# vkit-x/vkit

Measured on AMD Instinct MI355X. Metric: Mpixels/s (2048^2 RGB, geo+photo chain), higher is better.
Workload: dtype u8; 1 GPU; C3 fused chain: camera_cubic_curve remap (level 5) + gaussian_blur(sigma=1.0) + color_shift(37) + gaussion_noise(std=10.0, the numpy stream default_rng(5000 + i) drawn on the device inside every step), states built from the configs inside every step, 2048x2048x3 uint8, batch 256 per GPU; batch_per_gpu=256, image=2048x2048x3, noise_mode=tiles, states=built on the device from the configs inside every step (vkx_camera_states_dev), lanes=1

## Files before the change

vkit_amd/csrc/chain.hip:

```cpp
#include "vkx_internal.h"

#include <stdlib.h>
#include <algorithm>
#include <memory>
#include <unordered_map>
#include <vector>

static int chain_check_items(const vkx_chain_item *items, int n_items)
{
    for (int i = 0; i < n_items; i++) {
        const vkx_chain_item &it = items[i];
        VKX_REQUIRE(it.src && it.dst && it.src_vertices && it.dst_vertices, "NULL plane in chain item");
        VKX_REQUIRE(it.sh > 0 && it.sw > 0 && it.dh > 0 && it.dw > 0, "bad shape in chain item");
        VKX_REQUIRE_PITCH(it.src_stride, (ptrdiff_t)it.sw * 3, it.sh);
        VKX_REQUIRE_PITCH(it.dst_stride, (ptrdiff_t)it.dw * 3, it.dh);
        if (it.noise && !it.noise_tiled) VKX_REQUIRE_PITCH(it.noise_stride_el, (ptrdiff_t)it.dw * 3, it.dh);
        VKX_REQUIRE_DISJOINT(it.src, it.sh, it.src_stride, (size_t)it.sw * 3, it.dst, it.dh, it.dst_stride, (size_t)it.dw * 3);
        if (it.streak_enabled) {
            VKX_REQUIRE(it.streak_thickness + it.streak_gap > 0, "streak thickness + gap must be positive");
            if (it.streak_alpha < 0.0 || it.streak_alpha > 1.0) {
                vkx_set_error("alpha=%g is invalid.", it.streak_alpha);
                return VKX_ERR_INVALID;
            }
        }
// ... 112 lines not shown
        rc = vkx_chain_plan_build(ctx, items, n_items, &raw);
        if (rc && rc != VKX_ERR_UNSUPPORTED) return rc;
    }
    if (!raw) {
        if ((rc = vkx_chain_consume_lattices_mark(ctx))) return rc;
        if ((rc = vkx_np_draw_batch_dev(ctx, jobs, n_jobs, results_host))) return rc;
        return vkx_chain_rgb_batch_dev(ctx, items, n_items);
    }
    std::unique_ptr<vkx_chain_plan, void (*)(vkx_chain_plan *)> plan(raw, vkx_chain_plan_free);
    const int n_chunks = std::max(1, std::min(want_chunks, n_jobs / 8));
    struct Chunk { int job0, njobs, item0, nitems; vkx_np_chunk *np; hipEvent_t posted; };
    std::vector<Chunk> chunks((size_t)n_chunks);
    for (int c = 0; c < n_chunks; c++) {
        Chunk &ch = chunks[c];
        ch.job0 = (int)((long long)n_jobs * c / n_chunks);
        ch.njobs = (int)((long long)n_jobs * (c + 1) / n_chunks) - ch.job0;
        ch.item0 = c == 0 ? 0 : job_item[ch.job0];
        ch.np = nullptr; ch.posted = nullptr;
    }
    for (int c = 0; c < n_chunks; c++) chunks[c].nitems = (c + 1 < n_chunks ? chunks[c + 1].item0 : n_items) - chunks[c].item0;
    struct Cleanup {
        std::vector<Chunk> &chunks;
        ~Cleanup() { for (Chunk &ch : chunks) { if (ch.np) vkx_np_chunk_free(ch.np); if (ch.posted) (void)hipEventDestroy(ch.posted); } }
    } cleanup{chunks};

    vkx_device_guard guard(ctx);
    hipStream_t main_stream = ctx->stream;
    const char *fail_env = getenv("VKX_DEBUG_FAIL_CHUNK");
    const int fail_chunk = fail_env && fail_env[0] ? atoi(fail_env) : -1;
    auto schedule = [&]() -> int {
        int rc = VKX_OK;
        hipStream_t aux = vkx_stream_by_id(ctx, VKX_STREAM_COPY_IN, &rc);
        if (rc) return rc;
        hipEvent_t setup_done = nullptr;
        if ((rc = vkx_chain_plan_setup_aside(ctx, raw, &setup_done))) return rc;
        if (setup_done) VKX_HIP(hipStreamWaitEvent(aux, setup_done, 0));
        for (int c = 0; c < n_chunks; c++) {
            Chunk &ch = chunks[c];
            if (c >= 2) VKX_HIP(hipStreamWaitEvent(main_stream, chunks[c - 2].posted, 0));
            if ((rc = vkx_np_chunk_begin(ctx, jobs + ch.job0, ch.njobs, results_host + ch.job0, c & 1, &ch.np))) return rc;
            if ((rc = vkx_stream_order(ctx, aux, main_stream))) return rc;
            ctx->stream = aux;
            rc = vkx_np_chunk_finish(ctx, ch.np);
            if (!rc) rc = vkx_chain_plan_noise_rows(ctx, raw, ch.item0, ch.nitems);
            ctx->stream = main_stream;
            if (rc) return rc;
            VKX_HIP(hipEventCreateWithFlags(&ch.posted, hipEventDisableTiming));
            VKX_HIP(hipEventRecord(ch.posted, aux));
            if (c == fail_chunk) {
                vkx_set_error("injected failure in chunk %d (VKX_DEBUG_FAIL_CHUNK)", c);
                return VKX_ERR_INVALID;
            }
        }
        if (setup_done) VKX_HIP(hipStreamWaitEvent(main_stream, setup_done, 0));
        for (int c = 0; c < n_chunks; c++) {
            Chunk &ch = chunks[c];
            VKX_HIP(hipStreamWaitEvent(main_stream, ch.posted, 0));
            if ((rc = vkx_chain_plan_tiles(ctx, raw, ch.item0, ch.nitems))) return rc;
        }
        return vkx_chain_mark_done(ctx, main_stream);
    };
    rc = schedule();
    if (rc) vkx_ctx_join_streams(ctx, main_stream);
    return rc;
}
```

vkit_amd/csrc/ctx.hip:

```cpp
#include "vkx_internal.h"

#include <stdarg.h>
#include <stdio.h>

static thread_local char g_err[512] = "";

void vkx_set_error(const char *fmt, ...)
{
    va_list ap;
    va_start(ap, fmt);
    vsnprintf(g_err, sizeof g_err, fmt, ap);
    va_end(ap);
}

VKX_EXPORT const char *vkx_last_error(void) { return g_err; }
VKX_EXPORT int vkx_version(void) { return 1; }

VKX_EXPORT int vkx_device_count(int *count)
{
    VKX_REQUIRE(count != nullptr, "count is NULL");
    VKX_HIP(hipGetDeviceCount(count));
    return VKX_OK;
}

// ... 34 lines not shown

static void scratch_release(vkx_scratch *s)
{
    if (s->ptr) (void)hipFree(s->ptr);
    s->ptr = nullptr;
    s->cap = 0;
}

VKX_EXPORT int vkx_ctx_destroy(vkx_ctx *ctx)
{
    if (!ctx) return VKX_OK;
    (void)hipSetDevice(ctx->device);
    (void)hipStreamSynchronize(ctx->stream);
    for (auto &st : ctx->copy_stream)
        if (st) (void)hipStreamSynchronize(st);
    scratch_release(&ctx->owner);
    scratch_release(&ctx->paint_owner);
    scratch_release(&ctx->cells);
    scratch_release(&ctx->misc);
    scratch_release(&ctx->tables);
    for (auto &s : ctx->stage) scratch_release(&s);
    for (auto &s : ctx->chain) scratch_release(&s);
    scratch_release(&ctx->chain_cells);
    scratch_release(&ctx->chain_bins);
    scratch_release(&ctx->chain_misc);
    if (ctx->chain_done) (void)hipEventDestroy(ctx->chain_done);
    if (ctx->chain_setup_done) (void)hipEventDestroy(ctx->chain_setup_done);
    if (ctx->lattices_ready) (void)hipEventDestroy(ctx->lattices_ready);
    scratch_release(&ctx->noise_table);
    scratch_release(&ctx->np_tabs);
    scratch_release(&ctx->noise_rows);
    scratch_release(&ctx->np_work[0]);
    scratch_release(&ctx->np_work[1]);
    scratch_release(&ctx->camera_work);
    scratch_release(&ctx->mls_work);
    scratch_release(&ctx->fog_work);
    scratch_release(&ctx->crop_windows);
    scratch_release(&ctx->crop_planes);
    scratch_release(&ctx->combine_tables);
    scratch_release(&ctx->char_table);
    scratch_release(&ctx->char_geo);
    scratch_release(&ctx->char_layout);
    scratch_release(&ctx->char_host);
    scratch_release(&ctx->char_owner);
    scratch_release(&ctx->heat_table);
    scratch_release(&ctx->heat_geo);
    scratch_release(&ctx->heat_host);
    scratch_release(&ctx->heat_planes);
    scratch_release(&ctx->rl_deviate);
    scratch_release(&ctx->rl_planes);
    scratch_release(&ctx->rc_tables);
    scratch_release(&ctx->rc_bitmap);
    scratch_release(&ctx->rf_tables);
    scratch_release(&ctx->rm_tables);
    scratch_release(&ctx->rm_bits);
    scratch_release(&ctx->set_tables);
    scratch_release(&ctx->set_planes);
    scratch_release(&ctx->seal_tables);
    scratch_release(&ctx->seal_planes);
    scratch_release(&ctx->text_tables);
    scratch_release(&ctx->text_planes);
    scratch_release(&ctx->layer_tables);
    scratch_release(&ctx->quad_tables);
    scratch_release(&ctx->collate_tables);
    scratch_release(&ctx->contour_tables);
    scratch_release(&ctx->contour_planes);
// ... 560 lines not shown
```

vkit_amd/csrc/fused.hip:

```cpp
#include "vkx_internal.h"
#include "vkx_cell.h"
#include "vkx_color.h"

#include <float.h>
#include <memory>
#include <stdlib.h>
#include <string.h>

namespace {

constexpr int W = 64;
constexpr int RMAX = 3;
constexpr int NLDSCELL = 64;
#ifndef VKX_FUSED_NWAVES
#define VKX_FUSED_NWAVES 8
#endif
constexpr int NWAVES = VKX_FUSED_NWAVES;
constexpr int NTHREADS = 64 * NWAVES;
constexpr int ROWS_PER_WAVE = 8;
constexpr int WH = NWAVES * ROWS_PER_WAVE;
__host__ __device__ constexpr int tile_side(int R) { return (W - 2 * R) & ~3; }
__host__ __device__ constexpr int tile_height(int R) { return WH == W ? tile_side(R) : WH - 2 * R; }
#ifndef VKX_FUSED_CGROUP
#define VKX_FUSED_CGROUP 2
// ... 1114 lines not shown
    rec.y = before | (step << 16);
    ((u32x2 VKX_GLOBAL *)it.noise_rows)[k] = rec;
}

__global__ void __launch_bounds__(256) k_chain_prologue(uint32_t *__restrict__ desc_dst, const uint32_t *__restrict__ desc_src,
                                                        unsigned n_words, TileBin *__restrict__ bins, unsigned nbins,
                                                        int *__restrict__ deferred, int *__restrict__ over_count, unsigned n_over)
{
    const unsigned i = blockIdx.x * 256 + threadIdx.x;
    if (i < n_words) desc_dst[i] = desc_src[i];
    if (i < nbins) bins[i] = TileBin{0x7f7f7f7f, 0x7f7f7f7f, 0, 0};
    if (i < n_over) over_count[i] = 0;
    if (i == 0) *deferred = 0;
}

}

struct vkx_chain_plan {
    std::vector<ItemDev> dev;
    std::vector<int> prefix;
    std::vector<long long> row_prefix;
    long long ncells = 0;
    int max_tiles = 0, slots = 0;
    int rect_slots = 0;
    bool elements = false, streak = false;
    const ItemDev *d_items = nullptr;
    const int *d_cell_prefix = nullptr;
    TileBin *bins = nullptr;
    vkc::CellC *cells = nullptr;
    int *deferred = nullptr;
    int *over_count = nullptr;
    int2 *over_list = nullptr;
    const HsvLut *lut = nullptr;
};

void vkx_chain_plan_free(vkx_chain_plan *p) { delete p; }
int vkx_chain_plan_items(const vkx_chain_plan *p) { return (int)p->dev.size(); }

int vkx_chain_plan_setup(vkx_ctx *ctx, vkx_chain_plan *p)
{
    const int n_items = (int)p->dev.size();
    int rc;
    vkx_scratch *s_cells = p->elements ? &ctx->cells : &ctx->chain_cells;
    vkx_scratch *s_bins = p->elements ? &ctx->owner : &ctx->chain_bins;
    vkx_scratch *s_misc = p->elements ? &ctx->misc : &ctx->chain_misc;
    const size_t cells_bytes = sizeof(vkc::CellC) * (size_t)p->ncells;
    if ((rc = vkx_scratch_reserve(ctx, s_cells, cells_bytes + sizeof(int) * ((size_t)p->ncells + 1)))) return rc;
    p->slots = ((p->max_tiles + 7) / 8) * 8;
    const size_t nbins = (size_t)p->slots * n_items;
    if (n_items > 65535) return VKX_ERR_UNSUPPORTED;
    const size_t over_ints = p->elements ? 0 : (size_t)n_items * (2 + 2 * (size_t)p->rect_slots);
    if ((rc = vkx_scratch_reserve(ctx, s_bins, sizeof(TileBin) * nbins + sizeof(int) * over_ints))) return rc;
    const size_t items_bytes = sizeof(ItemDev) * (size_t)n_items, prefix_bytes = sizeof(int) * p->prefix.size();
    vkx_tables tab(ctx);
    const size_t items_off = tab.add(items_bytes), prefix_off = tab.add(prefix_bytes), misc_bytes = tab.bytes;
    if ((rc = vkx_scratch_reserve(ctx, s_misc, misc_bytes))) return rc;
    if (!p->elements && (rc = vkx_hsv_tables(ctx, (const void **)&p->lut))) return rc;
    unsigned char *misc = (unsigned char *)s_misc->ptr;
    if ((rc = tab.take())) return rc;
    memcpy(tab.at<char>(items_off), p->dev.data(), items_bytes);
    memcpy(tab.at<char>(prefix_off), p->prefix.data(), prefix_bytes);
    p->d_items = (const ItemDev *)(misc + items_off);
    p->d_cell_prefix = (const int *)(misc + prefix_off);
    p->bins = (TileBin *)s_bins->ptr;
    p->over_count = (int *)(p->bins + nbins);
    p->over_list = (int2 *)(p->over_count + n_items + (n_items & 1));
    p->cells = (vkc::CellC *)s_cells->ptr;
    p->deferred = (int *)((unsigned char *)s_cells->ptr + cells_bytes);
    {
        const unsigned char *ring_dev = tab.mapped();
        if (!ring_dev) { vkx_set_error("%s: the descriptor ring is not mapped into the device's address space", __func__); return VKX_ERR_HIP; }
        const size_t n_words = (misc_bytes + 3) / 4;
        VKX_TIMED(ctx, "k_chain_prologue");
        k_chain_prologue<<<vkx_blocks(std::max(n_words, nbins), 256), 256, 0, ctx->stream>>>((uint32_t *)misc, (const uint32_t *)ring_dev,
                                                                                            (unsigned)n_words, p->bins, (unsigned)nbins, p->deferred,
                                                                                            p->over_count, p->elements ? 0u : (unsigned)n_items);
        VKX_LAUNCH_CHECK();
    }
    { VKX_TIMED(ctx, "k_chain_setup"); k_chain_setup<<<vkx_blocks((size_t)p->ncells, 256), 256, 0, ctx->stream>>>(p->d_items, p->d_cell_prefix, n_items, (int)p->ncells, p->slots, p->cells, p->bins, p->deferred); }
    VKX_LAUNCH_CHECK();
    { VKX_TIMED(ctx, "k_chain_setup_svd"); k_chain_setup_svd<<<128, 64, 0, ctx->stream>>>(p->d_items, p->d_cell_prefix, n_items, p->cells, p->deferred); }
    VKX_LAUNCH_CHECK();
    return VKX_OK;
}

int vkx_chain_plan_noise_rows(vkx_ctx *ctx, vkx_chain_plan *p, int first, int count)
{
    if (p->row_prefix.empty() || count <= 0) return VKX_OK;
    long long most = 0;
    for (int i = first; i < first + count; i++) most = std::max(most, p->row_prefix[i + 1] - p->row_prefix[i]);
    if (most <= 0) return VKX_OK;
    VKX_TIMED(ctx, "k_chain_noise_rows");
    k_chain_noise_rows<<<dim3(vkx_blocks((size_t)most, 256), count), 256, 0, ctx->stream>>>(p->d_items + first);
    VKX_LAUNCH_CHECK();
    return VKX_OK;
}

int vkx_chain_plan_tiles(vkx_ctx *ctx, vkx_chain_plan *p, int first, int count)
{
    if (count <= 0) return VKX_OK;
    static const int phase_limit = vkx_env_int("VKX_FUSED_PHASES", 0);
    const ItemDev *items = p->d_items + first;
    const TileBin *bins = p->bins + (size_t)first * p->slots;
    if (p->elements) {
        const dim3 grid(p->slots, count);
        VKX_TIMED(ctx, "k_tile_remap");
        ElemPack pack;
        memset(&pack, 0, sizeof(pack));
        pack.n = p->dev[first].n_elems;
        for (int e = 0; e < 4; e++) pack.el[e] = p->dev[first].el[e];
        k_tile_remap<<<grid, NTHREADS, kFusedLds, ctx->stream>>>(items, p->cells, bins, pack);
    } else {
        int most_rect = 0, most_rim = 0;
        long long all_rect = 0, all_tiles = 0;
        for (int i = first; i < first + count; i++) {
            const ItemDev &d = p->dev[i];
            most_rect = std::max(most_rect, d.rect_w * d.rect_h);
            all_rect += d.rect_w * d.rect_h;
            all_tiles += (long long)d.tiles_x * d.tiles_y;
            most_rim = std::max(most_rim, d.tiles_x * d.tiles_y - d.rect_w * d.rect_h);
        }
        int *over_count = p->over_count + first;
        int2 *over_list = p->over_list + (size_t)first * p->rect_slots;
        const int over_slots = (int)std::min<long long>((long long)count * p->rect_slots, INT_MAX);
        VKX_TIMED_MAJOR(ctx, "k_chain_fused");
        constexpr long long kSplitMinTiles = 65536;
        const int split_env = vkx_env_on("VKX_CHAIN_SPLIT", -1);
        if (split_env >= 0 ? split_env == 0 : all_tiles < kSplitMinTiles) {
            const dim3 grid(p->slots, count);
            if (p->streak) k_chain_fused_whole<true><<<grid, NTHREADS, kFusedLds, ctx->stream>>>(items, p->cells, bins, p->lut, phase_limit);
            else k_chain_fused_whole<false><<<grid, NTHREADS, kFusedLds, ctx->stream>>>(items, p->cells, bins, p->lut, phase_limit);
            VKX_LAUNCH_CHECK();
            return VKX_OK;
        }
        if (most_rect > 0) {
            const dim3 grid_rect((most_rect + 7) / 8 * 8, count);
            if (p->streak) k_chain_fused<true><<<grid_rect, NTHREADS, kFusedLds, ctx->stream>>>(items, p->cells, bins, p->slots, over_count, over_list, over_slots, p->lut, phase_limit);
            else k_chain_fused<false><<<grid_rect, NTHREADS, kFusedLds, ctx->stream>>>(items, p->cells, bins, p->slots, over_count, over_list, over_slots, p->lut, phase_limit);
            VKX_LAUNCH_CHECK();
        }
        if (most_rim > 0) {
            const dim3 grid_rim((most_rim + 7) / 8 * 8, count);
            if (p->streak) k_chain_fused_rim<true><<<grid_rim, NTHREADS, kFusedLds, ctx->stream>>>(items, p->cells, bins, p->slots, p->lut, phase_limit);
            else k_chain_fused_rim<false><<<grid_rim, NTHREADS, kFusedLds, ctx->stream>>>(items, p->cells, bins, p->slots, p->lut, phase_limit);
            VKX_LAUNCH_CHECK();
        }
        if (most_rect > 0) {
            const dim3 grid_over((unsigned)std::min<long long>((all_rect + 1) / 2, kOverGrid));
            if (p->streak) k_chain_fused_over<true><<<grid_over, NTHREADS, kFusedLds, ctx->stream>>>(items, p->cells, bins, p->slots, over_count, over_list, over_slots, p->lut, phase_limit);
            else k_chain_fused_over<false><<<grid_over, NTHREADS, kFusedLds, ctx->stream>>>(items, p->cells, bins, p->slots, over_count, over_list, over_slots, p->lut, phase_limit);
        }
    }
    VKX_LAUNCH_CHECK();
    return VKX_OK;
}

int vkx_chain_plan_build(vkx_ctx *ctx, const vkx_chain_item *items, int n_items, vkx_chain_plan **out)
{
    *out = nullptr;
    if (n_items <= 0) return VKX_OK;
    std::unique_ptr<vkx_chain_plan> plan(new vkx_chain_plan());
    std::vector<ItemDev> &dev = plan->dev;
    dev.resize(n_items);
    plan->prefix.resize((size_t)n_items + 1);
    int *cell_prefix = plan->prefix.data();
    std::vector<long long> &row_prefix = plan->row_prefix;
    row_prefix.assign((size_t)n_items + 1, 0);
    long long tiles = 0, ncells = 0;
    int max_tiles = 0, max_rect = 0;
    for (int i = 0; i < n_items; i++) {
        const vkx_chain_item &it = items[i];
        if (it.blur_ksize > 2 * RMAX + 1 || (it.blur_ksize > 1 && (it.blur_ksize & 1) == 0)) return VKX_ERR_UNSUPPORTED;
        if (it.sh > 32767 || it.sw > 32767 || it.dh > 32767 || it.dw > 32767) return VKX_ERR_UNSUPPORTED;
        if (it.rows < 2 || it.cols < 2) return VKX_ERR_UNSUPPORTED;
        if (it.blur_ksize > 1 && (it.dh == 1 || it.dw == 1)) return VKX_ERR_UNSUPPORTED;
        ItemDev &d = dev[i];
        memset(&d, 0, sizeof(d));
        d.src = it.src; d.dst = it.dst; d.noise = it.noise; d.sv = it.src_vertices; d.dv = it.dst_vertices;
        d.sstride = it.src_stride; d.dstride = it.dst_stride; d.nstride = it.noise_stride_el;
        d.noise_table = nullptr; d.noise_tiled = 0; d.noise_tiles = 0; d.noise_slot = 0; d.noise_tiles_per_sample = 0.f;
        d.noise_rows = nullptr;
        if (it.noise && it.noise_tiled) {
            const long long n = (long long)it.dh * it.dw * 3;
            if (n > 0x7fffffffLL) return VKX_ERR_UNSUPPORTED;
            const vkx_np_tiles_shape shape = vkx_np_tiles_shape_of(n);
            if (shape.n_tiles * shape.slot_elems > 0xffffffffLL) return VKX_ERR_UNSUPPORTED;
            d.noise = (const int16_t *)((const unsigned char *)it.noise + shape.slots_offset);
// ... 157 lines not shown
```

vkit_amd/csrc/nprand.hip:

```cpp
#include "vkx_internal.h"
#include "np_ziggurat.h"
#include "vkx_host_tables.h"

#include <stddef.h>
#include <string.h>
#include <algorithm>

namespace {

typedef unsigned __int128 u128;
#define VKX_GLOBAL __attribute__((address_space(1)))

#ifndef VKX_NP_ROUNDS
#define VKX_NP_ROUNDS 48
#endif
constexpr int kRounds = VKX_NP_ROUNDS;
static_assert(kRounds % 2 == 0 && kRounds >= 2 && kRounds <= 64, "rounds per tile");
constexpr int kTile = 64 * kRounds;
constexpr double kNorR = 3.6541528853610087963519472518;
constexpr double kNorInvR = 0.27366123732975827203338247596;

#define PCG_MULT VKX_PCG_MULT
using vkx_host_tables::JumpTabs;

// ... 1223 lines not shown
    bool uniform, inline_jobs;
    long long total_tiles;
    vkx_np_result *results_host, *res_mapped;
    unsigned char *base;
    size_t o_states, o_info, o_plan, o_rmask, o_rval, o_jobs, o_results;
    NpJobPack pack;
    const NpTabs *tabs;
};

static int np_chunk_prepare(vkx_ctx *ctx, NpChunk &c)
{
    const bool uniform = c.uniform;
    c.total_tiles = 0;
    c.max_tiles = 0;
    for (int i = 0; i < c.n_jobs; i++) {
        const long long tiles = np_tiles_for(c.jobs[i], uniform);
        c.max_tiles = std::max<int>(c.max_tiles, (int)tiles);
        c.total_tiles += tiles;
    }
    size_t off = 0;
    auto take = [&off](size_t bytes) { const size_t o = off; off += vkx_align256(bytes); return o; };
    c.o_states = take((size_t)c.total_tiles * 16);
    c.o_info = take(uniform ? 0 : (size_t)c.total_tiles * sizeof(TileInfo));
    c.o_plan = take(uniform ? 0 : (size_t)c.total_tiles * sizeof(TilePlan));
    const bool speckle = c.kind == VKX_NP_SPECKLE_U8;
    const bool slots = c.kind == VKX_NP_NORMAL_I16 || c.kind == VKX_NP_NORMAL_ADD_U8;
    c.o_rmask = take(speckle ? (size_t)c.total_tiles * kRounds * 8 : 0);
    c.o_rval = take(speckle ? (size_t)c.total_tiles * kTile * 8 : slots ? (size_t)c.total_tiles * kSlot * 2 : 0);
    c.o_jobs = take((size_t)c.n_jobs * sizeof(NpJob));
    c.o_results = take((size_t)c.n_jobs * sizeof(vkx_np_result) + sizeof(unsigned));
    int rc = vkx_scratch_reserve(ctx, &ctx->np_work[c.slot], off);
    if (rc) return rc;
    c.base = (unsigned char *)ctx->np_work[c.slot].ptr;

    c.inline_jobs = c.n_jobs <= kInlineJobs;
    NpJob *hj = c.pack.jobs;
    vkx_tables tab(ctx);
    if (!c.inline_jobs) {
        if ((rc = tab.take((size_t)c.n_jobs * sizeof(NpJob)))) return rc;
        hj = tab.at<NpJob>(0);
    }
    const JumpTabs &jump = vkx_host_tables::jump_tabs();
    const u128 g64 = ((u128)jump.g64[1] << 64) | jump.g64[0];
    const u128 g128 = ((u128)jump.g128[1] << 64) | jump.g128[0];
    long long tile_base = 0;
    for (int i = 0; i < c.n_jobs; i++) {
        const vkx_np_job &j = c.jobs[i];
        NpJob &d = hj[i];
        d.state[0] = j.state[0]; d.state[1] = j.state[1];
        d.inc[0] = j.inc[0]; d.inc[1] = j.inc[1];
        const u128 c64 = (((u128)j.inc[1] << 64) | j.inc[0]) * g64;
        d.c64[0] = (uint64_t)c64; d.c64[1] = (uint64_t)(c64 >> 64);
        const u128 c128 = (((u128)j.inc[1] << 64) | j.inc[0]) * g128;
        d.c128[0] = (uint64_t)c128; d.c128[1] = (uint64_t)(c128 >> 64);
        d.n = j.n;
        d.tile_base = tile_base;
        d.n_tiles = (int)np_tiles_for(j, uniform);
        tile_base += d.n_tiles;
        d.kind = j.kind & 0xff; d.cn = j.cn;
        d.margin = (j.kind & VKX_NP_DEBUG_WIDE_MARGIN) ? 1.0 : 0x1p-42;
        d.loc = 0.0; d.scale = j.scale;
        d.cdf[0] = j.cdf[0]; d.cdf[1] = j.cdf[1]; d.cdf[2] = j.cdf[2];
        d.src = (const uint8_t *)j.src;
        d.dst = j.dst;
        d.rec = nullptr;
        d.table = nullptr;
        if (c.kind == VKX_NP_NORMAL_TILES) {
            const vkx_np_tiles_shape shape = vkx_np_tiles_shape_of(j.n);
            d.rec = (int16_t *)((unsigned char *)j.dst + shape.slots_offset);
            d.table = (uint2 *)((unsigned char *)j.dst + shape.table_offset);
        } else if (slots) {
            d.rec = (int16_t *)(c.base + c.o_rval) + d.tile_base * kSlot;
        }
    }
    if (!c.inline_jobs && (rc = tab.small_to(c.base + c.o_jobs))) return rc;
    c.res_mapped = nullptr;
    if (hipHostGetDevicePointer((void **)&c.res_mapped, c.results_host, 0) != hipSuccess) {
        (void)hipGetLastError();
        c.res_mapped = nullptr;
    }
    return VKX_OK;
}

static int np_chunk_front(vkx_ctx *ctx, NpChunk &c)
{
    unsigned char *base = c.base;
    const NpJob *dj = (const NpJob *)(base + c.o_jobs);
    uint64_t *states = (uint64_t *)(base + c.o_states);
    TileInfo *info = (TileInfo *)(base + c.o_info);
    vkx_np_result *res = (vkx_np_result *)(base + c.o_results);
    unsigned *done = (unsigned *)(res + c.n_jobs);
    const long long total_tiles = c.total_tiles;
    const int n_jobs = c.n_jobs, kind = c.kind;
    const NpTabs *tabs = c.tabs;
    static const int tpw_env = vkx_env_int("VKX_NP_TPW", 0);
    const int tiles_per_wave = tpw_env > 0 ? tpw_env : (total_tiles >= 160000 ? 4 : total_tiles >= 40000 ? 2 : 1);
    const unsigned wg = (unsigned)((total_tiles + 4 * tiles_per_wave - 1) / (4 * tiles_per_wave));
    {
        VKX_TIMED(ctx, "k_np_tile_states");
        if (c.inline_jobs)
            k_np_tile_states<true><<<vkx_blocks((size_t)total_tiles, 256), 256, 0, ctx->stream>>>(dj, c.pack, n_jobs, total_tiles, states, (NpJob *)(base + c.o_jobs), res, done, tabs);
        else
            k_np_tile_states<false><<<vkx_blocks((size_t)total_tiles, 256), 256, 0, ctx->stream>>>(dj, c.pack, n_jobs, total_tiles, states, (NpJob *)(base + c.o_jobs), res, done, tabs);
        VKX_LAUNCH_CHECK();
    }
    if (c.uniform) {
        VKX_TIMED(ctx, "k_np_choice_impulse");
        k_np_choice_impulse<<<wg, 256, 0, ctx->stream>>>(dj, n_jobs, total_tiles, states, res, done, c.res_mapped, tabs);
        VKX_LAUNCH_CHECK();
        return VKX_OK;
    }
    if (np_compact_records(kind)) {
        VKX_TIMED_MAJOR(ctx, "k_np_draw");
        bool bytes = true;
        for (int i = 0; i < n_jobs; i++) bytes = bytes && np_parks_as_bytes(c.jobs[i].scale, 0.0);
        const long long waves = bytes ? DrawShape<EmitI16B8>::kWaves : DrawShape<EmitI16>::kWaves;
        const unsigned wgc = (unsigned)((total_tiles + waves * tiles_per_wave - 1) / (waves * tiles_per_wave));
        const long long run = (total_tiles + (long long)wgc * waves - 1) / ((long long)wgc * waves);
        if (bytes)
            k_np_draw_compact<EmitI16B8><<<wgc, 64 * (unsigned)waves, 0, ctx->stream>>>(dj, n_jobs, total_tiles, run, states, info, res, tabs);
        else
            k_np_draw_compact<EmitI16><<<wgc, 64 * (unsigned)waves, 0, ctx->stream>>>(dj, n_jobs, total_tiles, run, states, info, res, tabs);
        VKX_LAUNCH_CHECK();
        return VKX_OK;
    }
    VKX_TIMED_MAJOR(ctx, "k_np_draw");
    k_np_draw<EmitSpeckle><<<wg, 256, 0, ctx->stream>>>(dj, n_jobs, total_tiles, states, info, (double *)(base + c.o_rval),
                                                        (uint64_t *)(base + c.o_rmask), res, tabs);
    VKX_LAUNCH_CHECK();
    return VKX_OK;
}

static int np_chunk_back(vkx_ctx *ctx, NpChunk &c)
{
    if (c.uniform) {
        if (!c.res_mapped)
            VKX_HIP(hipMemcpyAsync(c.results_host, c.base + c.o_results, (size_t)c.n_jobs * sizeof(vkx_np_result), hipMemcpyDeviceToHost, ctx->stream));
        return VKX_OK;
// ... 78 lines not shown
            VKX_REQUIRE(uniform, "normal and uniform jobs in one call");
            break;
        case VKX_NP_IMPULSE_U8:
            VKX_REQUIRE(uniform, "normal and uniform jobs in one call");
            VKX_REQUIRE(j.src != nullptr && j.cn >= 1 && j.cn <= 4, "bad impulse job");
            break;
        default:
            VKX_REQUIRE(false, "unknown job kind");
        }
        if (!uniform) VKX_REQUIRE(j.scale >= 0.0 && j.scale < 400.0, "scale outside [0, 400)");
        VKX_REQUIRE(np_tiles_for(j, uniform) <= 262144, "stream too long for one job (2.6e8 samples)");
    }
    return VKX_OK;
}

struct vkx_np_chunk { NpChunk c; };

int vkx_np_chunk_begin(vkx_ctx *ctx, const vkx_np_job *jobs, int n_jobs, vkx_np_result *results_host, int slot, vkx_np_chunk **out)
{
    *out = nullptr;
    const NpTabs *tabs = nullptr;
    int rc = np_tables(ctx, &tabs);
    if (rc) return rc;
    vkx_np_chunk *h = new (std::nothrow) vkx_np_chunk();
    if (!h) { vkx_set_error("out of host memory"); return VKX_ERR_NOMEM; }
    NpChunk &c = h->c;
    c.jobs = jobs; c.n_jobs = n_jobs;
    c.kind = jobs[0].kind & 0xff;
    c.uniform = c.kind == VKX_NP_CHOICE3_U8 || c.kind == VKX_NP_IMPULSE_U8;
    c.slot = slot & 1;
    c.results_host = results_host;
    c.tabs = tabs;
    vkx_device_guard guard(ctx);
    if ((rc = np_chunk_prepare(ctx, c)) || (rc = np_chunk_front(ctx, c))) { delete h; return rc; }
    *out = h;
    return VKX_OK;
}

int vkx_np_chunk_finish(vkx_ctx *ctx, vkx_np_chunk *h)
{
    vkx_device_guard guard(ctx);
    return np_chunk_back(ctx, h->c);
}

void vkx_np_chunk_free(vkx_np_chunk *h) { delete h; }

VKX_EXPORT int vkx_np_draw_batch_dev(vkx_ctx *ctx, const vkx_np_job *jobs, int n_jobs, vkx_np_result *results_host)
{
    VKX_REQUIRE(ctx && jobs && results_host, "NULL argument");
    int rc = vkx_np_jobs_check(jobs, n_jobs, results_host);
    if (rc) return rc;
    const int kind = jobs[0].kind & 0xff;
    const bool uniform = kind == VKX_NP_CHOICE3_U8 || kind == VKX_NP_IMPULSE_U8;
    const NpTabs *tabs = nullptr;
    if ((rc = np_tables(ctx, &tabs))) return rc;
    vkx_device_guard guard(ctx);
    const int n_chunks = (!uniform && kind != VKX_NP_NORMAL_TILES && n_jobs >= 2 * kChunkJobs) ? (n_jobs + kChunkJobs - 1) / kChunkJobs : 1;
    auto chunk_of = [&](int k, NpChunk &c) {
        const int per = (n_jobs + n_chunks - 1) / n_chunks, first = k * per;
        c.jobs = jobs + first;
        c.n_jobs = std::min(per, n_jobs - first);
        c.kind = kind; c.uniform = uniform; c.slot = k & 1;
        c.results_host = results_host + first;
        c.tabs = tabs;
    };
    if (n_chunks == 1) {
        NpChunk c;
        chunk_of(0, c);
        if ((rc = np_chunk_prepare(ctx, c)) || (rc = np_chunk_front(ctx, c))) return rc;
        return np_chunk_back(ctx, c);
    }
    hipStream_t main_stream = ctx->stream;
    hipStream_t aux = vkx_stream_by_id(ctx, VKX_STREAM_COPY_IN, &rc);
    if (rc) return rc;
    std::vector<hipEvent_t> placed(n_chunks, nullptr);
    for (int k = 0; k < n_chunks; k++) {
        NpChunk c;
        chunk_of(k, c);
        if (k >= 2) VKX_HIP(hipStreamWaitEvent(main_stream, placed[k - 2], 0));
        if ((rc = np_chunk_prepare(ctx, c)) || (rc = np_chunk_front(ctx, c))) return rc;
        if ((rc = vkx_stream_order(ctx, aux, main_stream))) return rc;
        ctx->stream = aux;
        rc = np_chunk_back(ctx, c);
        ctx->stream = main_stream;
        if (rc) return rc;
        VKX_HIP(hipEventCreateWithFlags(&placed[k], hipEventDisableTiming));
        VKX_HIP(hipEventRecord(placed[k], aux));
    }
    for (int k = std::max(0, n_chunks - 2); k < n_chunks; k++) VKX_HIP(hipStreamWaitEvent(main_stream, placed[k], 0));
    for (hipEvent_t e : placed) (void)hipEventDestroy(e);
    return VKX_OK;
}

VKX_EXPORT int vkx_np_tail_log_est_dev(vkx_ctx *ctx, const uint64_t *draws, int64_t n, double *est, double *eps)
{
    VKX_REQUIRE(ctx && draws && est, "NULL argument");
    VKX_REQUIRE(n >= 1 && n <= 0x7fffffffLL, "1 .. 2^31 - 1 draws");
    if (eps) *eps = kTailEps;
    vkx_device_guard guard(ctx);
    VKX_TIMED(ctx, "k_np_tail_log_est");
    k_np_tail_log_est<<<vkx_blocks((size_t)n, 256), 256, 0, ctx->stream>>>(draws, (long long)n, est);
    VKX_LAUNCH_CHECK();
    return VKX_OK;
}

VKX_EXPORT int vkx_np_draw(vkx_ctx *ctx, const vkx_np_job *job, vkx_np_result *result_host)
{
    VKX_REQUIRE(ctx && job && result_host, "NULL argument");
    VKX_REQUIRE(job->n >= 1 && job->n <= 0x7fffffffLL, "1 .. 2^31 - 1 samples per job");
    VKX_REQUIRE(job->dst != nullptr, "NULL destination");
    size_t src_bytes = 0, dst_bytes = 0;
    switch (job->kind & 0xff) {
    case VKX_NP_NORMAL_I16: dst_bytes = (size_t)job->n * 2; break;
// ... 41 lines not shown
```

vkit_amd/csrc/vkx_internal.h:

```cpp
#pragma once
#include <hip/hip_runtime.h>
#include <stdint.h>
#include <stddef.h>
#include <limits.h>
#include <stdlib.h>
#include <algorithm>
#include <cmath>
#include <string>
#include <utility>
#include <vector>

#include "../../include/vkx.h"

#define VKX_EXPORT extern "C" __attribute__((visibility("default")))

void vkx_set_error(const char *fmt, ...);

#define VKX_HIP(call)                                                                      \
    do {                                                                                   \
        hipError_t e__ = (call);                                                           \
        if (e__ != hipSuccess) {                                                           \
            vkx_set_error("%s failed: %s (%s:%d)", #call, hipGetErrorString(e__), __FILE__, \
                          __LINE__);                                                       \
            return VKX_ERR_HIP;                                                            \
// ... 77 lines not shown
            return VKX_ERR_HIP;                                              \
        }                                                                    \
    } while (0)

struct vkx_scratch {
    void *ptr = nullptr;
    size_t cap = 0;
};

struct vkx_ctx {
    int device = 0;
    hipStream_t own_stream = nullptr;
    hipStream_t stream = nullptr;
    vkx_scratch owner;
    vkx_scratch paint_owner;
    size_t paint_owner_zeroed = 0;
    vkx_scratch cells;
    vkx_scratch misc;
    vkx_scratch tables;
    bool tables_ready = false;
    vkx_scratch stage[2];
    vkx_scratch chain[3];
    vkx_scratch chain_cells, chain_bins, chain_misc;
    hipEvent_t chain_setup_done = nullptr;
    hipEvent_t chain_done = nullptr;
    hipEvent_t lattices_ready = nullptr;
    bool lattices_armed = false;
    vkx_scratch noise_table;
    double noise_table_std = 0.0;
    bool noise_table_fits8 = false;
    vkx_scratch np_tabs;
    vkx_scratch noise_rows;
    vkx_scratch np_work[2];
    vkx_scratch mls_work;
    vkx_scratch camera_work;
    vkx_scratch fog_work;
    vkx_scratch jpeg_planes;
    vkx_scratch crop_windows, crop_planes;
    vkx_scratch combine_tables;
    vkx_scratch char_table, char_geo, char_layout, char_host;
    vkx_scratch char_owner;
    size_t char_owner_zeroed = 0;
    vkx_scratch heat_table, heat_geo, heat_host;
    vkx_scratch heat_planes;
    size_t heat_clean_page = 0;
    vkx_scratch rl_deviate, rl_planes;
    vkx_scratch rc_tables, rc_bitmap;
    vkx_scratch rf_tables;
    vkx_scratch rm_tables, rm_bits;
    vkx_scratch set_tables, set_planes;
    vkx_scratch seal_tables, seal_planes;
    vkx_scratch text_tables, text_planes;
    vkx_scratch layer_tables;
    vkx_scratch quad_tables;
    vkx_scratch collate_tables;
    vkx_scratch contour_tables, contour_planes;
    vkx_scratch ov_tables, ov_bits;
    vkx_scratch glass_win;
    vkx_scratch pz_tabs, pz_work, pz_draws;
    bool pz_tabs_ready = false;

    hipStream_t copy_stream[2] = {nullptr, nullptr};
    std::vector<hipEvent_t> order_events;
    unsigned char *desc_ring = nullptr;
    size_t desc_cap = 0, desc_off = 0;
    int desc_hold = 0;
// ... 242 lines not shown
    double d = at(0, 0) * (at(1, 1) * at(2, 2) - at(1, 2) * at(2, 1)) -
               at(0, 1) * (at(1, 0) * at(2, 2) - at(1, 2) * at(2, 0)) +
               at(0, 2) * (at(1, 0) * at(2, 1) - at(1, 1) * at(2, 0));
    if (d == 0.) {
        for (int i = 0; i < 9; i++) c.m[i] = 0;
    } else {
        d = 1. / d;
        c.m[0] = (at(1, 1) * at(2, 2) - at(1, 2) * at(2, 1)) * d;
        c.m[1] = (at(0, 2) * at(2, 1) - at(0, 1) * at(2, 2)) * d;
        c.m[2] = (at(0, 1) * at(1, 2) - at(0, 2) * at(1, 1)) * d;
        c.m[3] = (at(1, 2) * at(2, 0) - at(1, 0) * at(2, 2)) * d;
        c.m[4] = (at(0, 0) * at(2, 2) - at(0, 2) * at(2, 0)) * d;
        c.m[5] = (at(0, 2) * at(1, 0) - at(0, 0) * at(1, 2)) * d;
        c.m[6] = (at(1, 0) * at(2, 1) - at(1, 1) * at(2, 0)) * d;
        c.m[7] = (at(0, 1) * at(2, 0) - at(0, 0) * at(2, 1)) * d;
        c.m[8] = (at(0, 0) * at(1, 1) - at(0, 1) * at(1, 0)) * d;
    }
    const int BLOCK_SZ = 32;
    const int bh0 = BLOCK_SZ / 2 < dh ? BLOCK_SZ / 2 : (dh > 0 ? dh : 1);
    c.bw0 = BLOCK_SZ * BLOCK_SZ / bh0 < dw ? BLOCK_SZ * BLOCK_SZ / bh0 : (dw > 0 ? dw : 1);
    return c;
}

}

int vkx_hsv_tables(vkx_ctx *ctx, const void **out);
int vkx_gaussian_kernel_q8_host(int n, double sigma, uint16_t *kq);
int vkx_chain_fused_try(vkx_ctx *ctx, const vkx_chain_item *items, int n_items);
struct vkx_chain_plan;
int vkx_chain_plan_build(vkx_ctx *ctx, const vkx_chain_item *items, int n_items, vkx_chain_plan **out);
void vkx_chain_plan_free(vkx_chain_plan *p);
int vkx_chain_plan_setup_aside(vkx_ctx *ctx, vkx_chain_plan *p, hipEvent_t *done);
int vkx_chain_plan_noise_rows(vkx_ctx *ctx, vkx_chain_plan *p, int first, int count);
int vkx_chain_plan_tiles(vkx_ctx *ctx, vkx_chain_plan *p, int first, int count);
int vkx_chain_mark_done(vkx_ctx *ctx, hipStream_t stream);
struct vkx_np_chunk;
int vkx_np_jobs_check(const vkx_np_job *jobs, int n_jobs, const vkx_np_result *results_host);
int vkx_np_chunk_begin(vkx_ctx *ctx, const vkx_np_job *jobs, int n_jobs, vkx_np_result *results_host, int slot, vkx_np_chunk **out);
int vkx_np_chunk_finish(vkx_ctx *ctx, vkx_np_chunk *c);
void vkx_np_chunk_free(vkx_np_chunk *c);
int vkx_tile_remap_try(vkx_ctx *ctx, const vkx_elem *elems, int n_elems, int sh, int sw, const int32_t *src_vertices,
                       const int32_t *dst_vertices, int rows, int cols, int dh, int dw);
struct vkx_np_tiles_shape {
    long long n_tiles;
    int slot_elems;
    size_t table_offset, slots_offset, bytes;
    double samples_per_tile;
};
vkx_np_tiles_shape vkx_np_tiles_shape_of(long long n);
```

Before: 78430 Mpixels/s.

## Overlap noise RNG state setup, tile waits and over-pass across streams

```diff
diff --git a/vkit_amd/csrc/chain.hip b/vkit_amd/csrc/chain.hip
--- a/vkit_amd/csrc/chain.hip
+++ b/vkit_amd/csrc/chain.hip
@@ -168,14 +168,33 @@
         int rc = VKX_OK;
         hipStream_t aux = vkx_stream_by_id(ctx, VKX_STREAM_COPY_IN, &rc);
         if (rc) return rc;
+        hipStream_t side = vkx_stream_by_id(ctx, VKX_STREAM_COPY_OUT, &rc);
+        if (rc) return rc;
+        const int n_ahead = n_chunks >= 2 ? 1 : 0;
+        if (n_ahead) {
+            if (ctx->np_drawn_armed) {
+                VKX_HIP(hipStreamWaitEvent(side, ctx->np_drawn, 0));
+                VKX_HIP(hipStreamWaitEvent(side, ctx->np_posted, 0));
+            } else if ((rc = vkx_stream_order(ctx, side, main_stream)) || (rc = vkx_stream_order(ctx, side, aux))) return rc;
+            ctx->stream = side;
+            rc = vkx_np_chunk_begin(ctx, jobs + chunks[0].job0, chunks[0].njobs, results_host + chunks[0].job0, 0, &chunks[0].np);
+            ctx->stream = main_stream;
+            if (rc) return rc;
+            if ((rc = vkx_stream_order(ctx, main_stream, side))) return rc;
+        }
         hipEvent_t setup_done = nullptr;
         if ((rc = vkx_chain_plan_setup_aside(ctx, raw, &setup_done))) return rc;
         if (setup_done) VKX_HIP(hipStreamWaitEvent(aux, setup_done, 0));
         for (int c = 0; c < n_chunks; c++) {
             Chunk &ch = chunks[c];
             if (c >= 2) VKX_HIP(hipStreamWaitEvent(main_stream, chunks[c - 2].posted, 0));
-            if ((rc = vkx_np_chunk_begin(ctx, jobs + ch.job0, ch.njobs, results_host + ch.job0, c & 1, &ch.np))) return rc;
-            if ((rc = vkx_stream_order(ctx, aux, main_stream))) return rc;
+            if (c >= n_ahead && (rc = vkx_np_chunk_begin(ctx, jobs + ch.job0, ch.njobs, results_host + ch.job0, c & 1, &ch.np))) return rc;
+            if ((rc = vkx_np_chunk_draw(ctx, ch.np))) return rc;
+            if (c == n_chunks - 1) {
+                if (!ctx->np_drawn) VKX_HIP(hipEventCreateWithFlags(&ctx->np_drawn, hipEventDisableTiming));
+                VKX_HIP(hipEventRecord(ctx->np_drawn, main_stream));
+                VKX_HIP(hipStreamWaitEvent(aux, ctx->np_drawn, 0));
+            } else if ((rc = vkx_stream_order(ctx, aux, main_stream))) return rc;
             ctx->stream = aux;
             rc = vkx_np_chunk_finish(ctx, ch.np);
             if (!rc) rc = vkx_chain_plan_noise_rows(ctx, raw, ch.item0, ch.nitems);
@@ -188,12 +207,16 @@
                 return VKX_ERR_INVALID;
             }
         }
-        if (setup_done) VKX_HIP(hipStreamWaitEvent(main_stream, setup_done, 0));
+        if (!ctx->np_posted) VKX_HIP(hipEventCreateWithFlags(&ctx->np_posted, hipEventDisableTiming));
+        VKX_HIP(hipEventRecord(ctx->np_posted, aux));
+        ctx->np_drawn_armed = true;
+        vkx_chain_plan_over_aside(raw, aux);
+        VKX_HIP(hipStreamWaitEvent(main_stream, chunks[0].posted, 0));
         for (int c = 0; c < n_chunks; c++) {
             Chunk &ch = chunks[c];
-            VKX_HIP(hipStreamWaitEvent(main_stream, ch.posted, 0));
-            if ((rc = vkx_chain_plan_tiles(ctx, raw, ch.item0, ch.nitems))) return rc;
-        }
+            if ((rc = vkx_chain_plan_tiles(ctx, raw, ch.item0, ch.nitems, c + 1 < n_chunks ? chunks[c + 1].posted : nullptr))) return rc;
+        }
+        if ((rc = vkx_chain_plan_join_over(ctx, raw, main_stream))) return rc;
         return vkx_chain_mark_done(ctx, main_stream);
     };
     rc = schedule();
diff --git a/vkit_amd/csrc/ctx.hip b/vkit_amd/csrc/ctx.hip
--- a/vkit_amd/csrc/ctx.hip
+++ b/vkit_amd/csrc/ctx.hip
@@ -90,6 +90,8 @@
     scratch_release(&ctx->noise_rows);
     scratch_release(&ctx->np_work[0]);
     scratch_release(&ctx->np_work[1]);
+    if (ctx->np_drawn) (void)hipEventDestroy(ctx->np_drawn);
+    if (ctx->np_posted) (void)hipEventDestroy(ctx->np_posted);
     scratch_release(&ctx->camera_work);
     scratch_release(&ctx->mls_work);
     scratch_release(&ctx->fog_work);
diff --git a/vkit_amd/csrc/fused.hip b/vkit_amd/csrc/fused.hip
--- a/vkit_amd/csrc/fused.hip
+++ b/vkit_amd/csrc/fused.hip
@@ -1170,9 +1170,12 @@
     int *over_count = nullptr;
     int2 *over_list = nullptr;
     const HsvLut *lut = nullptr;
+    hipStream_t over_stream = nullptr;
+    bool over_pending = false;
 };
 
 void vkx_chain_plan_free(vkx_chain_plan *p) { delete p; }
+void vkx_chain_plan_over_aside(vkx_chain_plan *p, hipStream_t stream) { p->over_stream = stream; }
 int vkx_chain_plan_items(const vkx_chain_plan *p) { return (int)p->dev.size(); }
 
 int vkx_chain_plan_setup(vkx_ctx *ctx, vkx_chain_plan *p)
@@ -1234,9 +1237,12 @@
     return VKX_OK;
 }
 
-int vkx_chain_plan_tiles(vkx_ctx *ctx, vkx_chain_plan *p, int first, int count)
-{
-    if (count <= 0) return VKX_OK;
+int vkx_chain_plan_tiles(vkx_ctx *ctx, vkx_chain_plan *p, int first, int count, hipEvent_t then_wait)
+{
+    if (count <= 0) {
+        if (then_wait) { vkx_device_guard guard(ctx); VKX_HIP(hipStreamWaitEvent(ctx->stream, then_wait, 0)); }
+        return VKX_OK;
+    }
     static const int phase_limit = vkx_env_int("VKX_FUSED_PHASES", 0);
     const ItemDev *items = p->d_items + first;
     const TileBin *bins = p->bins + (size_t)first * p->slots;
@@ -1248,6 +1254,7 @@
         pack.n = p->dev[first].n_elems;
         for (int e = 0; e < 4; e++) pack.el[e] = p->dev[first].el[e];
         k_tile_remap<<<grid, NTHREADS, kFusedLds, ctx->stream>>>(items, p->cells, bins, pack);
+        if (then_wait) VKX_HIP(hipStreamWaitEvent(ctx->stream, then_wait, 0));
     } else {
         int most_rect = 0, most_rim = 0;
         long long all_rect = 0, all_tiles = 0;
@@ -1269,6 +1276,7 @@
             if (p->streak) k_chain_fused_whole<true><<<grid, NTHREADS, kFusedLds, ctx->stream>>>(items, p->cells, bins, p->lut, phase_limit);
             else k_chain_fused_whole<false><<<grid, NTHREADS, kFusedLds, ctx->stream>>>(items, p->cells, bins, p->lut, phase_limit);
             VKX_LAUNCH_CHECK();
+            if (then_wait) VKX_HIP(hipStreamWaitEvent(ctx->stream, then_wait, 0));
             return VKX_OK;
         }
         if (most_rect > 0) {
@@ -1277,6 +1285,13 @@
             else k_chain_fused<false><<<grid_rect, NTHREADS, kFusedLds, ctx->stream>>>(items, p->cells, bins, p->slots, over_count, over_list, over_slots, p->lut, phase_limit);
             VKX_LAUNCH_CHECK();
         }
+        hipStream_t over_stream = ctx->stream;
+        if (most_rect > 0 && most_rim > 0 && p->over_stream && p->over_stream != ctx->stream) {
+            over_stream = p->over_stream;
+            int orc = vkx_stream_order(ctx, over_stream, ctx->stream);
+            if (orc) return orc;
+        }
+        if (then_wait) VKX_HIP(hipStreamWaitEvent(ctx->stream, then_wait, 0));
         if (most_rim > 0) {
             const dim3 grid_rim((most_rim + 7) / 8 * 8, count);
             if (p->streak) k_chain_fused_rim<true><<<grid_rim, NTHREADS, kFusedLds, ctx->stream>>>(items, p->cells, bins, p->slots, p->lut, phase_limit);
@@ -1285,12 +1300,22 @@
         }
         if (most_rect > 0) {
             const dim3 grid_over((unsigned)std::min<long long>((all_rect + 1) / 2, kOverGrid));
-            if (p->streak) k_chain_fused_over<true><<<grid_over, NTHREADS, kFusedLds, ctx->stream>>>(items, p->cells, bins, p->slots, over_count, over_list, over_slots, p->lut, phase_limit);
-            else k_chain_fused_over<false><<<grid_over, NTHREADS, kFusedLds, ctx->stream>>>(items, p->cells, bins, p->slots, over_count, over_list, over_slots, p->lut, phase_limit);
+            if (over_stream != ctx->stream) p->over_pending = true;
+            if (p->streak) k_chain_fused_over<true><<<grid_over, NTHREADS, kFusedLds, over_stream>>>(items, p->cells, bins, p->slots, over_count, over_list, over_slots, p->lut, phase_limit);
+            else k_chain_fused_over<false><<<grid_over, NTHREADS, kFusedLds, over_stream>>>(items, p->cells, bins, p->slots, over_count, over_list, over_slots, p->lut, phase_limit);
         }
     }
     VKX_LAUNCH_CHECK();
     return VKX_OK;
+}
+
+int vkx_chain_plan_join_over(vkx_ctx *ctx, vkx_chain_plan *p, hipStream_t stream)
+{
+    if (!p->over_pending) return VKX_OK;
+    vkx_device_guard guard(ctx);
+    int rc = vkx_stream_order(ctx, stream, p->over_stream);
+    if (!rc) p->over_pending = false;
+    return rc;
 }
 
 int vkx_chain_plan_build(vkx_ctx *ctx, const vkx_chain_item *items, int n_items, vkx_chain_plan **out)
diff --git a/vkit_amd/csrc/nprand.hip b/vkit_amd/csrc/nprand.hip
--- a/vkit_amd/csrc/nprand.hip
+++ b/vkit_amd/csrc/nprand.hip
@@ -1279,6 +1279,7 @@
     int rc = vkx_scratch_reserve(ctx, &ctx->np_work[c.slot], off);
     if (rc) return rc;
     c.base = (unsigned char *)ctx->np_work[c.slot].ptr;
+    ctx->np_drawn_armed = false;
 
     c.inline_jobs = c.n_jobs <= kInlineJobs;
     NpJob *hj = c.pack.jobs;
@@ -1329,7 +1330,26 @@
     return VKX_OK;
 }
 
-static int np_chunk_front(vkx_ctx *ctx, NpChunk &c)
+static int np_chunk_states(vkx_ctx *ctx, NpChunk &c)
+{
+    unsigned char *base = c.base;
+    const NpJob *dj = (const NpJob *)(base + c.o_jobs);
+    uint64_t *states = (uint64_t *)(base + c.o_states);
+    vkx_np_result *res = (vkx_np_result *)(base + c.o_results);
+    unsigned *done = (unsigned *)(res + c.n_jobs);
+    const long long total_tiles = c.total_tiles;
+    const int n_jobs = c.n_jobs;
+    const NpTabs *tabs = c.tabs;
+    VKX_TIMED(ctx, "k_np_tile_states");
+    if (c.inline_jobs)
+        k_np_tile_states<true><<<vkx_blocks((size_t)total_tiles, 256), 256, 0, ctx->stream>>>(dj, c.pack, n_jobs, total_tiles, states, (NpJob *)(base + c.o_jobs), res, done, tabs);
+    else
+        k_np_tile_states<false><<<vkx_blocks((size_t)total_tiles, 256), 256, 0, ctx->stream>>>(dj, c.pack, n_jobs, total_tiles, states, (NpJob *)(base + c.o_jobs), res, done, tabs);
+    VKX_LAUNCH_CHECK();
+    return VKX_OK;
+}
+
+static int np_chunk_draw(vkx_ctx *ctx, NpChunk &c)
 {
     unsigned char *base = c.base;
     const NpJob *dj = (const NpJob *)(base + c.o_jobs);
@@ -1343,14 +1363,6 @@
     static const int tpw_env = vkx_env_int("VKX_NP_TPW", 0);
     const int tiles_per_wave = tpw_env > 0 ? tpw_env : (total_tiles >= 160000 ? 4 : total_tiles >= 40000 ? 2 : 1);
     const unsigned wg = (unsigned)((total_tiles + 4 * tiles_per_wave - 1) / (4 * tiles_per_wave));
-    {
-        VKX_TIMED(ctx, "k_np_tile_states");
-        if (c.inline_jobs)
-            k_np_tile_states<true><<<vkx_blocks((size_t)total_tiles, 256), 256, 0, ctx->stream>>>(dj, c.pack, n_jobs, total_tiles, states, (NpJob *)(base + c.o_jobs), res, done, tabs);
-        else
-            k_np_tile_states<false><<<vkx_blocks((size_t)total_tiles, 256), 256, 0, ctx->stream>>>(dj, c.pack, n_jobs, total_tiles, states, (NpJob *)(base + c.o_jobs), res, done, tabs);
-        VKX_LAUNCH_CHECK();
-    }
     if (c.uniform) {
         VKX_TIMED(ctx, "k_np_choice_impulse");
         k_np_choice_impulse<<<wg, 256, 0, ctx->stream>>>(dj, n_jobs, total_tiles, states, res, done, c.res_mapped, tabs);
@@ -1495,9 +1507,15 @@
     c.results_host = results_host;
     c.tabs = tabs;
     vkx_device_guard guard(ctx);
-    if ((rc = np_chunk_prepare(ctx, c)) || (rc = np_chunk_front(ctx, c))) { delete h; return rc; }
+    if ((rc = np_chunk_prepare(ctx, c)) || (rc = np_chunk_states(ctx, c))) { delete h; return rc; }
     *out = h;
     return VKX_OK;
+}
+
+int vkx_np_chunk_draw(vkx_ctx *ctx, vkx_np_chunk *h)
+{
+    vkx_device_guard guard(ctx);
+    return np_chunk_draw(ctx, h->c);
 }
 
 int vkx_np_chunk_finish(vkx_ctx *ctx, vkx_np_chunk *h)
@@ -1530,7 +1548,7 @@
     if (n_chunks == 1) {
         NpChunk c;
         chunk_of(0, c);
-        if ((rc = np_chunk_prepare(ctx, c)) || (rc = np_chunk_front(ctx, c))) return rc;
+        if ((rc = np_chunk_prepare(ctx, c)) || (rc = np_chunk_states(ctx, c)) || (rc = np_chunk_draw(ctx, c))) return rc;
         return np_chunk_back(ctx, c);
     }
     hipStream_t main_stream = ctx->stream;
@@ -1541,7 +1559,7 @@
         NpChunk c;
         chunk_of(k, c);
         if (k >= 2) VKX_HIP(hipStreamWaitEvent(main_stream, placed[k - 2], 0));
-        if ((rc = np_chunk_prepare(ctx, c)) || (rc = np_chunk_front(ctx, c))) return rc;
+        if ((rc = np_chunk_prepare(ctx, c)) || (rc = np_chunk_states(ctx, c)) || (rc = np_chunk_draw(ctx, c))) return rc;
         if ((rc = vkx_stream_order(ctx, aux, main_stream))) return rc;
         ctx->stream = aux;
         rc = np_chunk_back(ctx, c);
diff --git a/vkit_amd/csrc/vkx_internal.h b/vkit_amd/csrc/vkx_internal.h
--- a/vkit_amd/csrc/vkx_internal.h
+++ b/vkit_amd/csrc/vkx_internal.h
@@ -133,6 +133,9 @@
     vkx_scratch np_tabs;
     vkx_scratch noise_rows;
     vkx_scratch np_work[2];
+    hipEvent_t np_drawn = nullptr;
+    hipEvent_t np_posted = nullptr;
+    bool np_drawn_armed = false;
     vkx_scratch mls_work;
     vkx_scratch camera_work;
     vkx_scratch fog_work;
@@ -441,11 +444,14 @@
 void vkx_chain_plan_free(vkx_chain_plan *p);
 int vkx_chain_plan_setup_aside(vkx_ctx *ctx, vkx_chain_plan *p, hipEvent_t *done);
 int vkx_chain_plan_noise_rows(vkx_ctx *ctx, vkx_chain_plan *p, int first, int count);
-int vkx_chain_plan_tiles(vkx_ctx *ctx, vkx_chain_plan *p, int first, int count);
+int vkx_chain_plan_tiles(vkx_ctx *ctx, vkx_chain_plan *p, int first, int count, hipEvent_t then_wait = nullptr);
+void vkx_chain_plan_over_aside(vkx_chain_plan *p, hipStream_t stream);
+int vkx_chain_plan_join_over(vkx_ctx *ctx, vkx_chain_plan *p, hipStream_t stream);
 int vkx_chain_mark_done(vkx_ctx *ctx, hipStream_t stream);
 struct vkx_np_chunk;
 int vkx_np_jobs_check(const vkx_np_job *jobs, int n_jobs, const vkx_np_result *results_host);
 int vkx_np_chunk_begin(vkx_ctx *ctx, const vkx_np_job *jobs, int n_jobs, vkx_np_result *results_host, int slot, vkx_np_chunk **out);
+int vkx_np_chunk_draw(vkx_ctx *ctx, vkx_np_chunk *c);
 int vkx_np_chunk_finish(vkx_ctx *ctx, vkx_np_chunk *c);
 void vkx_np_chunk_free(vkx_np_chunk *c);
 int vkx_tile_remap_try(vkx_ctx *ctx, const vkx_elem *elems, int n_elems, int sh, int sw, const int32_t *src_vertices,
```

After: 78910 Mpixels/s (median of 6 runs). Within noise of the previous version (+0.6%).
